# cherubicXN/neat

Measured on AMD Instinct MI355X. Metric: ray-samples/s (train step) on ABC-neat-a, higher is better.
Workload: dtype bf16; 1 GPU; C2: abc-neat-a networks, 1024 rays x 128 samples per GPU, depth samples given, train step = forward + loss + backward + Adam; rays_per_gpu=1024, samples_per_ray=128, global_rays=1024, parallelism=dp1, weights=synthetic 'rough' (seed 42), launch=hip graph replay, the whole step one launch (forward + loss + backward + Adam)

## Files before the change

neat_amd/csrc/kernels_bf16.hpp:

```cpp
#pragma once
#include "kernels.hpp"
#include "bf16_common.hpp"

namespace neat {

__device__ __forceinline__ size_t oct_index(int f, int p, int ldp) { return ((size_t)(f >> 3) * ldp + p) * 8 + (f & 7); }

struct SegH { const void* p; int rows; int bf16; };

struct LayerArgsH {
  SegH in[2];
  int Kpad;
  const uint4* Wp;
  const float* bias;
  int bias_rot, bias_n;
  int N, NT;
  int ldp;
  void* out0; void* out1;
  int out0_bf16, out1_bf16, n_split, accumulate;
  const u16* aux0; const u16* aux1;
  const u16* padfill_oct;
  const float* padfill; int padfill_rows;
};

// ... 626 lines not shown
      if (fast) {
        const int p = pb + bpg * 8;
        uint4 raw[8];
#pragma unroll
        for (int t = 0; t < 8; ++t) raw[t] = (okr && p + t < pend) ? rawl[t * 64 + lane] : make_uint4(0u, 0u, 0u, 0u);
        w2_transpose(raw, blk);
      } else {
        w2_rows_f32(pr, isA, row0, pb + bpg * 8, a.ldp, pend, blk);
      }
      unsigned char* dst = (isA ? As : Bs) + (boct * 8) * HLD + bpg * 16;
#pragma unroll
      for (int f = 0; f < 8; ++f) *reinterpret_cast<uint4*>(dst + f * HLD) = blk[f];
      if (bias_now) {
#pragma unroll
        for (int f = 0; f < 8; ++f) {
          const unsigned w4[4] = {blk[f].x, blk[f].y, blk[f].z, blk[f].w};
          float t = 0.0f;
#pragma unroll
          for (int j = 0; j < 4; ++j) t += bf_lo(w4[j]) + bf_hi(w4[j]);
          rsum[f] += t;
        }
      }
      __syncthreads();
      if (st + 1 < nsteps) W2_ISSUE(pr, pb + HBP);
      else if (q == 0 && a.npairs > 1) W2_ISSUE(a.pair[1], pbeg);
      const unsigned char* ap = As + (wr + (lane & 31)) * HLD + (lane >> 5) * 16;
      const unsigned char* bp = Bs + (wc + (lane & 31)) * HLD + (lane >> 5) * 16;
#pragma unroll
      for (int s = 0; s < HBP / 16; ++s) {
        uint4 av[2], bv[4];
#pragma unroll
        for (int i = 0; i < 2; ++i) av[i] = *reinterpret_cast<const uint4*>(ap + i * 32 * HLD + s * 32);
#pragma unroll
        for (int j = 0; j < 4; ++j) bv[j] = *reinterpret_cast<const uint4*>(bp + j * 32 * HLD + s * 32);
#pragma unroll
        for (int i = 0; i < 2; ++i) {
          if (!liveR[i]) continue;
#pragma unroll
          for (int j = 0; j < 4; ++j)
            if (liveC[j])
              acc[i][j] = NEAT_MFMA16(*reinterpret_cast<bf16x8*>(&av[i]), *reinterpret_cast<bf16x8*>(&bv[j]), acc[i][j], 0, 0, 0);
        }
      }
      __syncthreads();
    }
  }
#undef W2_ISSUE
#undef W2_SEG
#undef W2_FAST
  float* dstp = a.partial + (size_t)blockIdx.y * a.split_stride;
#pragma unroll
  for (int i = 0; i < 2; ++i) {
    if (!liveR[i]) continue;
#pragma unroll
    for (int r = 0; r < 16; ++r) {
      const int n = n0 + wr + 32 * i + (r & 3) + 8 * (r >> 2) + 4 * (lane >> 5);
      if (n >= a.N) continue;
#pragma unroll
      for (int j = 0; j < 4; ++j) {
        const int k = k0 + wc + 32 * j + (lane & 31);
        if (liveC[j] && k < a.Kt) dstp[(size_t)n * a.row_stride + k] = acc[i][j][r];
      }
    }
  }
  if (do_bias && isA) {
#pragma unroll
    for (int f = 0; f < 8; ++f) {
      float v = rsum[f];
      v += __shfl_xor(v, 1); v += __shfl_xor(v, 2); v += __shfl_xor(v, 4);
      if (bpg == 0 && row0 + f < a.N) dstp[(size_t)(row0 + f) * a.row_stride + a.bias_col] = v;
    }
  }
}

struct OctPackJob { const float* src; int rows; u16* dst; };
struct OctPackArgs { OctPackJob job[4]; int njobs, ldp; };
__global__ void oct_pack_kernel(OctPackArgs a) {
  const int p = blockIdx.x * blockDim.x + threadIdx.x;
  if (p >= a.ldp) return;
#pragma unroll
  for (int j = 0; j < 4; ++j) {
    if (j >= a.njobs) break;
    const OctPackJob jb = a.job[j];
    for (int o = 0; o * 8 < jb.rows; ++o) {
      float v[8];
#pragma unroll
      for (int e = 0; e < 8; ++e) v[e] = (o * 8 + e < jb.rows) ? jb.src[(size_t)(o * 8 + e) * a.ldp + p] : 0.0f;
      reinterpret_cast<uint4*>(jb.dst)[(size_t)o * a.ldp + p] = make_uint4(pack2(v[0], v[1]), pack2(v[2], v[3]), pack2(v[4], v[5]), pack2(v[6], v[7]));
    }
  }
}

struct BwdPrologueArgs {
  const float* sc_r; const float* sc_a; const float* extra_rm; const float* mask; const float* d_tail_rm;
  const float* cot_slot; const float* cot_slot_a;
  int P, ldp, P_main;
  const float* x_fm; const float* E;
  float* gh; float* Eh;
  u16* Ebf; u16* Ebf4; u16* Ehbf; u16* Ehbf4;
  const float* dbeta_ray; int R; const float* beta_ptr; float* dbeta;
};
__global__ __launch_bounds__(256) void bwd_prologue_kernel(BwdPrologueArgs a) {
  if (a.dbeta && blockIdx.x == gridDim.x - 1) { beta_grad_body(a.dbeta_ray, a.R, a.beta_ptr, a.dbeta); return; }
  const int p = blockIdx.x * blockDim.x + threadIdx.x;
  if (p >= a.ldp) return;
  const size_t ldp = (size_t)a.ldp;
  const float ext_scale = cot_scale_of(a.cot_slot);
  const float rho_a = a.cot_slot_a ? ext_scale / cot_scale_of(a.cot_slot_a) : 1.0f;
  const float keep = (p < a.P) ? 1.0f - (a.mask ? a.mask[p] : 0.0f) : 0.0f;
  float eh[40], ev[40];
#pragma unroll
  for (int c = 0; c < 3; ++c) {
    float v = 0.0f;
    if (p < a.P_main) {
      if (a.sc_r) v += a.sc_r[(size_t)(30 + c) * ldp + p];
      if (a.sc_a) v += a.sc_a[(size_t)(6 + c) * ldp + p] * rho_a;
      if (a.extra_rm) v += a.extra_rm[p * 3 + c] * ext_scale;
    } else if (p < a.P && a.d_tail_rm) {
      v = a.d_tail_rm[(p - a.P_main) * 3 + c] * ext_scale;
    }
    const float gc = v * keep;
    a.gh[(size_t)c * ldp + p] = gc;
    const float xc = a.x_fm[(size_t)c * ldp + p];
    eh[c] = gc;
    float f = 1.0f;
#pragma unroll
    for (int k = 0; k < 6; ++k) {
      eh[3 + 6 * k + c] = f * __cosf(xc * f) * gc;
      eh[6 + 6 * k + c] = -f * __sinf(xc * f) * gc;
      f *= 2.0f;
    }
  }
  eh[39] = 0.0f; ev[39] = 0.0f;
#pragma unroll
  for (int j = 0; j < 39; ++j) { a.Eh[(size_t)j * ldp + p] = eh[j]; ev[j] = a.E[(size_t)j * ldp + p]; }
  auto octet = [](const float (&v)[40], int r0) {
    float t[8];
#pragma unroll
    for (int e = 0; e < 8; ++e) t[e] = (r0 + e < 39) ? v[r0 + e] : 0.0f;
    return make_uint4(pack2(t[0], t[1]), pack2(t[2], t[3]), pack2(t[4], t[5]), pack2(t[6], t[7]));
  };
#pragma unroll
  for (int o = 0; o < 5; ++o) {
    reinterpret_cast<uint4*>(a.Ebf)[(size_t)o * ldp + p] = octet(ev, 8 * o);
    reinterpret_cast<uint4*>(a.Ehbf)[(size_t)o * ldp + p] = octet(eh, 8 * o);
  }
#pragma unroll
  for (int o = 0; o < 4; ++o) {
    reinterpret_cast<uint4*>(a.Ebf4)[(size_t)o * ldp + p] = octet(ev, 7 + 8 * o);
    reinterpret_cast<uint4*>(a.Ehbf4)[(size_t)o * ldp + p] = octet(eh, 7 + 8 * o);
  }
}

#ifndef NEAT_W3_ABLATE
#define NEAT_W3_ABLATE 0
#endif
constexpr int W3T = 512, W3P = 32, W3NS = 4;
template <int NCB> struct W3Cfg {
  static constexpr int QA = 8, QB = 2 * NCB;
  static constexpr int STAGE = (QA + QB) * 2048;
  static constexpr int LDS = W3NS * STAGE;
  static constexpr int QPW = NCB == 5 ? 3 : 2;
  static constexpr int G = 2 * QPW;
};
constexpr int W3_STAGE = W3Cfg<4>::STAGE;
constexpr int W3_LDS_BYTES = W3Cfg<4>::LDS;
constexpr int W3_SLOTS = 12;
struct WgradArgsH3 {
  const unsigned short* A[W3_SLOTS]; const unsigned short* B[W3_SLOTS]; int rowsA[W3_SLOTS];
  const unsigned short* B2[W3_SLOTS];
  int splitB, octsB;
  int npairs, N, K, P, ldp, chunk;
  float* partial; size_t row_stride, split_stride; int col_off, bias_col;
  int nt_loads;
  int interleave;
  int nprob; size_t prob_stride;
};
typedef short v4s16 __attribute__((ext_vector_type(4)));

template <int NCB>
__global__ __launch_bounds__(W3T, 2) void wgrad_kernel_h3(WgradArgsH3 a) {
  typedef W3Cfg<NCB> C;
  extern __shared__ __attribute__((aligned(16))) unsigned char w3lds[];
  typedef __attribute__((address_space(3))) void* lds_ptr;
  typedef __attribute__((address_space(3))) v4s16* lds_v4;
  typedef const __attribute__((address_space(1))) void* gbl_ptr;
  const int tid = threadIdx.x, lane = tid & 63, wave = tid >> 6;
  const int wr = (wave >> 1) * 64, wc = (wave & 1) * 32 * NCB;
  const int nsplit = gridDim.y;
  const int pstep = a.interleave ? nsplit * W3P : W3P;
  const int pbeg = a.interleave ? blockIdx.y * W3P : blockIdx.y * a.chunk;
  const int pend = a.interleave ? a.P : min(a.P, pbeg + a.chunk);
  const int nsteps = a.interleave ? ((a.P + W3P - 1) / W3P - (int)blockIdx.y + nsplit - 1) / nsplit : (pend - pbeg + W3P - 1) / W3P;
  const int prob = a.nprob > 1 ? (int)blockIdx.x : 0;
  const int T = nsteps * a.npairs;
  bool liveR[2], liveC[NCB];
#pragma unroll
  for (int i = 0; i < 2; ++i) liveR[i] = wr + 32 * i < a.N;
#pragma unroll
  for (int j = 0; j < NCB; ++j) liveC[j] = wc + 32 * j < a.K;
  f32x16 acc[2][NCB];
#pragma unroll
  for (int i = 0; i < 2; ++i)
#pragma unroll
    for (int j = 0; j < NCB; ++j)
#pragma unroll
      for (int r = 0; r < 16; ++r) acc[i][j][r] = 0.0f;
  float rsum[2] = {0.0f, 0.0f};

  const int dl_oct = lane & 3, dl_pt = lane >> 2;
  const unsigned lds_base = (unsigned)(size_t)(lds_ptr)w3lds;
  const unsigned short* opbase[2][C::QPW]; const unsigned short* opbase2[2]; int opmax[2][C::QPW]; int opq[C::QPW]; bool opB[C::QPW];
#pragma unroll
  for (int hq = 0; hq < C::QPW; ++hq) {
    const int g = min(C::QPW * wave + hq, C::QA + C::QB - 1);
    opB[hq] = g >= C::QA; opq[hq] = opB[hq] ? g - C::QA : g;
  }
#pragma unroll
  for (int q = 0; q < 2; ++q) {
    const int idx = prob * a.npairs + q;
    const unsigned short* pA = a.A[0]; const unsigned short* pB = a.B[0]; const unsigned short* p2 = a.B2[0];
    int rA = a.rowsA[0];
#pragma unroll
    for (int k = 1; k < W3_SLOTS; ++k)
      if (idx == k) { pA = a.A[k]; pB = a.B[k]; p2 = a.B2[k]; rA = a.rowsA[k]; }
    opbase2[q] = p2;
#pragma unroll
    for (int hq = 0; hq < C::QPW; ++hq) { opbase[q][hq] = opB[hq] ? pB : pA; opmax[q][hq] = opB[hq] ? a.octsB - 1 : (rA + 7) / 8 - 1; }
  }
  auto issue = [&](int tau) {
    const int q = tau >= nsteps ? 1 : 0;
    const int st = tau - q * nsteps;
    if (NEAT_W3_ABLATE == 4) return;
    const unsigned short* base2 = q ? opbase2[1] : opbase2[0];
    const unsigned stage = lds_base + (tau % W3NS) * C::STAGE;
#pragma unroll
    for (int hq = 0; hq < C::QPW; ++hq) {
      const unsigned short* base = q ? opbase[1][hq] : opbase[0][hq];
      const int maxoct = q ? opmax[1][hq] : opmax[0][hq];
      const int oct = min(4 * opq[hq] + dl_oct, maxoct);
      const bool second = opB[hq] && oct >= a.splitB;
      const uint4* seg = reinterpret_cast<const uint4*>(second ? base2 : base) + (size_t)(second ? oct - a.splitB : oct) * a.ldp;
      const int g = min(C::QPW * wave + hq, C::QA + C::QB - 1);
#ifndef NEAT_W3_SKIP_SURPLUS
#define NEAT_W3_SKIP_SURPLUS 1
#endif
      if constexpr (NEAT_W3_SKIP_SURPLUS && 8 * C::QPW > C::QA + C::QB) { if (C::QPW * wave + hq >= C::QA + C::QB) continue; }
#pragma unroll
      for (int i = 0; i < 2; ++i) {
        const int p = pbeg + st * pstep + 16 * i + dl_pt;
        const uint4* src = seg + p;
        const unsigned dst = __builtin_amdgcn_readfirstlane(stage + g * 2048 + i * 1024);
        unsigned keep;
        if (a.nt_loads)
          asm volatile("s_mov_b32 %0, m0\n\ts_mov_b32 m0, %2\n\ts_nop 0\n\tglobal_load_lds_dwordx4 %1, off nt\n\ts_mov_b32 m0, %0"
                       : "=&s"(keep) : "v"(src), "s"(dst) : "memory");
        else
          asm volatile("s_mov_b32 %0, m0\n\ts_mov_b32 m0, %2\n\ts_nop 0\n\tglobal_load_lds_dwordx4 %1, off\n\ts_mov_b32 m0, %0"
                       : "=&s"(keep) : "v"(src), "s"(dst) : "memory");
      }
    }
  };
#pragma unroll
  for (int t = 0; t < W3NS - 1; ++t)
    if (t < T) issue(t);

  const int G = lane >> 4, li = lane & 15;
  const int frag_off = ((8 * (G >> 1) + (li >> 2)) * 64) + (G & 1) * 32 + (li & 3) * 8;
  const bool do_bias = a.bias_col >= 0 && wc == 0;

  for (int tau = 0; tau < T; ++tau) {
    if (tau + 2 < T) { if (C::G == 4) asm volatile("s_waitcnt vmcnt(8)\n\ts_barrier" ::: "memory"); else asm volatile("s_waitcnt vmcnt(12)\n\ts_barrier" ::: "memory"); }
    else if (tau + 1 < T) { if (C::G == 4) asm volatile("s_waitcnt vmcnt(4)\n\ts_barrier" ::: "memory"); else asm volatile("s_waitcnt vmcnt(6)\n\ts_barrier" ::: "memory"); }
    else asm volatile("s_waitcnt vmcnt(0)\n\ts_barrier" ::: "memory");
    if (tau + W3NS - 1 < T) issue(tau + W3NS - 1);
    const unsigned char* slot = w3lds + (tau % W3NS) * C::STAGE;
    const int st = tau >= nsteps ? tau - nsteps : tau;
    const int pb = pbeg + st * pstep;
    const bool tail = pb + W3P > pend;
    const bool bias_now = do_bias && tau < nsteps;
#pragma unroll
    for (int s2 = 0; s2 < W3P / 16; ++s2) {
      uint4 av[2], bv[NCB];
#pragma unroll
      for (int i = 0; i < 2; ++i) {
        if (NEAT_W3_ABLATE == 2) { av[i] = make_uint4(lane, tau, i, s2); continue; }
        const unsigned char* ap = slot + ((wr >> 5) + i) * 2048 + s2 * 1024 + frag_off;
        const v4s16 lo = __builtin_amdgcn_ds_read_tr16_b64_v4i16((lds_v4)(ap));
        const v4s16 hi = __builtin_amdgcn_ds_read_tr16_b64_v4i16((lds_v4)(ap + 256));
        av[i] = make_uint4(((const unsigned*)&lo)[0], ((const unsigned*)&lo)[1], ((const unsigned*)&hi)[0], ((const unsigned*)&hi)[1]);
      }
#pragma unroll
      for (int j = 0; j < NCB; ++j) {
        if (NEAT_W3_ABLATE == 2) { bv[j] = make_uint4(lane, tau, j, s2); continue; }
        const unsigned char* bp = slot + C::QA * 2048 + ((wc >> 5) + j) * 2048 + s2 * 1024 + frag_off;
        const v4s16 lo = __builtin_amdgcn_ds_read_tr16_b64_v4i16((lds_v4)(bp));
        const v4s16 hi = __builtin_amdgcn_ds_read_tr16_b64_v4i16((lds_v4)(bp + 256));
        bv[j] = make_uint4(((const unsigned*)&lo)[0], ((const unsigned*)&lo)[1], ((const unsigned*)&hi)[0], ((const unsigned*)&hi)[1]);
      }
      if (tail) {
        const int p0 = pb + 16 * s2 + 8 * (G >> 1);
        auto mask4 = [&](uint4& v) {
          unsigned w4[4] = {v.x, v.y, v.z, v.w};
#pragma unroll
          for (int e = 0; e < 4; ++e) {
            const bool k0 = p0 + 2 * e < pend, k1 = p0 + 2 * e + 1 < pend;
            w4[e] = (k0 ? (w4[e] & 0x0000FFFFu) : 0u) | (k1 ? (w4[e] & 0xFFFF0000u) : 0u);
          }
          v = make_uint4(w4[0], w4[1], w4[2], w4[3]);
        };
#pragma unroll
        for (int i = 0; i < 2; ++i) mask4(av[i]);
#pragma unroll
        for (int j = 0; j < NCB; ++j) mask4(bv[j]);
      }
      if (bias_now) {
#pragma unroll
        for (int i = 0; i < 2; ++i) {
          const unsigned w4[4] = {av[i].x, av[i].y, av[i].z, av[i].w};
          float t = rsum[i];
#pragma unroll
          for (int e = 0; e < 4; ++e) { t += bf_lo(w4[e]); t += bf_hi(w4[e]); }
          asm volatile("" : "+v"(t));
          rsum[i] = t;
        }
      }
#pragma unroll
      for (int i = 0; i < 2; ++i) {
        if (!liveR[i]) continue;
#pragma unroll
        for (int j = 0; j < NCB; ++j)
          if (liveC[j]) {
            if (NEAT_W3_ABLATE == 1) { asm volatile("" :: "v"(av[i].x), "v"(av[i].w), "v"(bv[j].x), "v"(bv[j].w)); continue; }
            acc[i][j] = NEAT_MFMA16(*reinterpret_cast<bf16x8*>(&av[i]), *reinterpret_cast<bf16x8*>(&bv[j]), acc[i][j], 0, 0, 0);
          }
      }
    }
  }
  float* dstp = a.partial + (size_t)prob * a.prob_stride + (size_t)blockIdx.y * a.split_stride;
  auto put = [&](float* q, float v) {
    if (NEAT_W3_ABLATE == 3 && v != 123.0f) return;
    *q = v;
  };
#pragma unroll
  for (int i = 0; i < 2; ++i) {
    if (!liveR[i]) continue;
#pragma unroll
    for (int r = 0; r < 16; ++r) {
      const int n = wr + 32 * i + (r & 3) + 8 * (r >> 2) + 4 * (lane >> 5);
      if (n >= a.N) continue;
#pragma unroll
      for (int j = 0; j < NCB; ++j) {
        const int k = wc + 32 * j + (lane & 31);
        if (liveC[j] && k < a.K) put(dstp + (size_t)n * a.row_stride + a.col_off + k, acc[i][j][r]);
      }
    }
  }
  if (do_bias) {
#pragma unroll
    for (int i = 0; i < 2; ++i) {
      float v = rsum[i];
      v += __shfl_xor(v, 32);
      const int n = wr + 32 * i + (lane & 31);
      if (lane < 32 && n < a.N) put(dstp + (size_t)n * a.row_stride + a.bias_col, v);
    }
  }
}

struct PackDesc2 {
  int layer, transpose, N, K, Kpad, NT;
  int s0, s0p, off0, off1;
  int rot;
  float scale; int offset; int blk0; int bf16;
  int lo;
};
constexpr int MAXPACKS2 = 48;
struct PackArgs2 { NetPtrs net; const float* rowscale; int row_off[NLAYERS + 1]; PackDesc2 d[MAXPACKS2]; int npacks; float* out; };

__device__ __forceinline__ float packed_weight(const PackDesc2& d, const float* v, const float* rs, int O, int I, int n, int k) {
  if (!v || n >= d.N || k >= d.K) return 0.0f;
  const int po = d.transpose ? k : n;
  const int pj = d.transpose ? n : k;
  if (po >= O) return 0.0f;
  const int o = (po + d.rot) % O;
  int i;
  if (pj < d.s0p) { if (pj >= d.s0) return 0.0f; i = d.off0 + pj; }
  else { i = d.off1 + (pj - d.s0p); if (pj - d.s0p >= I - d.s0) return 0.0f; }
  if (i >= I) return 0.0f;
  return v[(size_t)o * I + i] * rs[o] * d.scale;
}

__global__ __launch_bounds__(WG) void pack_kernel2(PackArgs2 a) {
  int pk = 0;
  while (pk + 1 < a.npacks && (int)blockIdx.x >= a.d[pk + 1].blk0) ++pk;
  const PackDesc2 d = a.d[pk];
  const int nt = blockIdx.x - d.blk0;
  const int O = a.net.O[d.layer], I = a.net.I[d.layer];
  const float* v = a.net.v[d.layer];
  const float* rs = a.rowscale + a.row_off[d.layer];
  if (d.bf16) {
    const int KS = d.Kpad >> 4;
    uint4* out = reinterpret_cast<uint4*>(a.out + d.offset) + (size_t)nt * KS * 64;
    for (int e = blockIdx.y * WG + threadIdx.x; e < KS * 64; e += WG * gridDim.y) {
      const int s = e >> 6, ln = e & 63;
      const int n = nt * 32 + (ln & 31), kb = 16 * s + 8 * (ln >> 5);
      float w[8];
#pragma unroll
      for (int t = 0; t < 8; ++t) w[t] = packed_weight(d, v, rs, O, I, n, kb + t);
      if (d.lo) {
#pragma unroll
        for (int t = 0; t < 8; ++t) w[t] -= bf2f(f2bf(w[t]));
      }
      out[e] = make_uint4(pack2(w[0], w[1]), pack2(w[2], w[3]), pack2(w[4], w[5]), pack2(w[6], w[7]));
    }
  } else {
    const int KS = d.Kpad >> 1;
    float* out = a.out + d.offset + (size_t)nt * KS * 64;
    for (int e = blockIdx.y * WG + threadIdx.x; e < KS * 64; e += WG * gridDim.y) {
      const int s = e >> 6, ln = e & 63;
      out[e] = packed_weight(d, v, rs, O, I, nt * 32 + (ln & 31), 2 * s + (ln >> 5));
    }
  }
}

__global__ void adjoint_seed_kernel_h(const float* __restrict__ v8, const float* __restrict__ rs8, const u16* __restrict__ h8,
                                      int ldp, u16* __restrict__ u7) {
  const int p = blockIdx.x * blockDim.x + threadIdx.x;
  const int oct = blockIdx.y;
  if (p >= ldp) return;
  const size_t idx = ((size_t)oct * ldp + p) * 8;
  const uint4 hv = *reinterpret_cast<const uint4*>(h8 + idx);
  const unsigned hw[4] = {hv.x, hv.y, hv.z, hv.w};
  unsigned o[4];
#pragma unroll
  for (int j = 0; j < 4; ++j) {
    const float w0 = v8[oct * 8 + 2 * j] * rs8[0], w1 = v8[oct * 8 + 2 * j + 1] * rs8[0];
    o[j] = pack2(w0 * dphi_fast(bf_lo(hw[j])), w1 * dphi_fast(bf_hi(hw[j])));
  }
  *reinterpret_cast<uint4*>(u7 + idx) = make_uint4(o[0], o[1], o[2], o[3]);
}

__global__ void oct_to_rm_kernel(const u16* __restrict__ src, int P, int C, int ldp, float* __restrict__ dst, int ldc, int col0,
                                 const u16* __restrict__ srclo = nullptr) {
  const int p = blockIdx.x * blockDim.x + threadIdx.x, o = blockIdx.y;
  if (p >= P) return;
  const uint4 v = reinterpret_cast<const uint4*>(src)[(size_t)o * ldp + p];
  uint4 vl = make_uint4(0u, 0u, 0u, 0u);
  if (srclo) vl = reinterpret_cast<const uint4*>(srclo)[(size_t)o * ldp + p];
  const unsigned w4[4] = {v.x, v.y, v.z, v.w}, l4[4] = {vl.x, vl.y, vl.z, vl.w};
  float* d = dst + (size_t)p * ldc + col0 + o * 8;
#pragma unroll
  for (int j = 0; j < 4; ++j) {
    if (o * 8 + 2 * j < C) d[2 * j] = bf_lo(w4[j]) + bf_lo(l4[j]);
    if (o * 8 + 2 * j + 1 < C) d[2 * j + 1] = bf_hi(w4[j]) + bf_hi(l4[j]);
  }
}
__global__ void export_out8_kernel(const float* __restrict__ sdfraw, const u16* __restrict__ src, const u16* __restrict__ srclo, int P, int ldp,
                                   float* __restrict__ out257, float* __restrict__ feat) {
  const int p = blockIdx.x * blockDim.x + threadIdx.x, o = blockIdx.y;
  if (p >= P) return;
  const uint4 v = reinterpret_cast<const uint4*>(src)[(size_t)o * ldp + p];
  uint4 vl = make_uint4(0u, 0u, 0u, 0u);
  if (srclo) vl = reinterpret_cast<const uint4*>(srclo)[(size_t)o * ldp + p];
  const unsigned w4[4] = {v.x, v.y, v.z, v.w}, l4[4] = {vl.x, vl.y, vl.z, vl.w};
  float f[8];
#pragma unroll
  for (int j = 0; j < 4; ++j) { f[2 * j] = bf_lo(w4[j]) + bf_lo(l4[j]); f[2 * j + 1] = bf_hi(w4[j]) + bf_hi(l4[j]); }
  if (out257) {
    float* d = out257 + (size_t)p * 257 + 1 + o * 8;
#pragma unroll
    for (int j = 0; j < 8; ++j) d[j] = f[j];
    if (o == 0) out257[(size_t)p * 257] = sdfraw[p];
  }
  if (feat) {
    float* d = feat + (size_t)p * 256 + o * 8;
#pragma unroll
    for (int j = 0; j < 8; ++j) d[j] = f[j];
  }
}
__global__ void rm_to_oct_kernel(const float* __restrict__ src, int P, int C, int ldp, u16* __restrict__ dst, u16* __restrict__ dstlo = nullptr) {
  const int p = blockIdx.x * blockDim.x + threadIdx.x;
  if (p >= ldp) return;
  const int Cp = (C + 7) & ~7;
  for (int c = 0; c < Cp; ++c) {
    const float v = (p < P && c < C) ? src[(size_t)p * C + c] : 0.0f;
    const u16 h = f2bf(v);
    dst[oct_index(c, p, ldp)] = h;
    if (dstlo) dstlo[oct_index(c, p, ldp)] = f2bf(v - bf2f(h));
  }
}
__global__ void fm_col_to_rm_kernel(const float* __restrict__ src, int P, float* __restrict__ dst, int ldc, int col) {
  const int p = blockIdx.x * blockDim.x + threadIdx.x;
  if (p < P) dst[(size_t)p * ldc + col] = src[p];
}
// ... 3 lines not shown
```

neat_amd/csrc/kernels_dw.hpp:

```cpp
#pragma once
#include "kernels_bf16.hpp"

namespace neat {

struct LayerArgsDW {
  LayerArgsWS w;
  const u16* auxA2; int auxA_split;
  int rowsA;
  int P;
  uint4* partial;
  float* pscale;
  float* pbias;
  int ablate;
};

constexpr int DW_MAXSEG = 4;
struct LayerArgsDWSeg { LayerArgsDW l[DW_MAXSEG]; int n; };

constexpr int DW_XLDS = 1024;
constexpr int DW_WG_UINT4 = 8 * 8 * 2 * 64;
#ifndef DW_VALU_PER_MFMA
#define DW_VALU_PER_MFMA 14
#endif

// ... 149 lines not shown
          dacc[i * 4 + j] = NEAT_MFMA16(*reinterpret_cast<const bf16x8*>(&av[i]), *reinterpret_cast<const bf16x8*>(&bv[j]), dacc[i * 4 + j], 0, 0, 0);
    };
    f32x16 acc;
    auto chain = [&]() {
#pragma unroll
      for (int r = 0; r < 16; ++r) acc[r] = 0.0f;
      const unsigned bfrag_e = (hi5 * WSP + (l31 ^ (hi5 << 2))) * 16;
      const unsigned bfrag_o = (hi5 * WSP + (l31 ^ ((2 + hi5) << 2))) * 16;
#pragma unroll
      for (int ks = 0; ks < 16; ++ks) {
        const uint4 bv = *reinterpret_cast<const uint4*>(slot + ((ks & 1) ? bfrag_o : bfrag_e) + ks * (2 * WSP * 16));
        acc = NEAT_MFMA16(*reinterpret_cast<const bf16x8*>(&wreg[ks]), *reinterpret_cast<const bf16x8*>(&bv), acc, 0, 0, 0);
      }
    };
    const int p = tile * WSP + (int)l31;
    auto epi_half = [&](int j, bool fullrows, const uint4* fa = nullptr, const uint4* fb = nullptr) {
      float sp = 0.0f;
      if (C::HAS_S) sp = *reinterpret_cast<const float*>(slot + EXTRA + wave * 256 + l31 * 4);
      uint2 pk0[2], pk1[2];
#pragma unroll
      for (int qq = 0; qq < 2; ++qq) {
        const int q = 2 * j + qq;
        pk0[qq] = make_uint2(0u, 0u); pk1[qq] = make_uint2(0u, 0u);
        const int n0 = wave * 32 + 8 * q + 4 * (int)hi5;
        if (!fullrows && fa) {
#pragma unroll
          for (int e = 0; e < 4; ++e) {
            const int t = qq * 4 + e;
            dacc[t] = NEAT_MFMA16(*reinterpret_cast<const bf16x8*>(&fa[t >> 2]), *reinterpret_cast<const bf16x8*>(&fb[t & 3]), dacc[t], 0, 0, 0);
          }
        }
        if (!fullrows && wave * 32 + 8 * q >= Npad) continue;
        const unsigned eoff = dma_off + q * (WSP * 16) + ((l31 ^ ((unsigned)q << 2)) * 16) + hi5 * 8;
        const uint2 r0v = *reinterpret_cast<const uint2*>(slot + AUX0 + eoff);
        const uint2 r1v = *reinterpret_cast<const uint2*>(slot + AUX1 + eoff);
        const float x0[4] = {bf_lo(r0v.x), bf_hi(r0v.x), bf_lo(r0v.y), bf_hi(r0v.y)};
        const float x1[4] = {bf_lo(r1v.x), bf_hi(r1v.x), bf_lo(r1v.y), bf_hi(r1v.y)};
        float o0[4], o1[4];
        float4 b8 = make_float4(0.f, 0.f, 0.f, 0.f);
        if (EPI == EPI_BWD8) b8 = *reinterpret_cast<const float4*>(w8 + n0);
        const float bias8q[4] = {b8.x, b8.y, b8.z, b8.w};
#pragma unroll
        for (int e = 0; e < 4; ++e) {
          const float v = acc[4 * q + e];
          if (fa && fullrows) {
            const int t = qq * 4 + e;
            dacc[t] = NEAT_MFMA16(*reinterpret_cast<const bf16x8*>(&fa[t >> 2]), *reinterpret_cast<const bf16x8*>(&fb[t & 3]), dacc[t], 0, 0, 0);
          }
          float r0 = 0.0f, r1 = 0.0f;
          if (TANK) { const float sg = dphi_fast(x0[e]); r0 = v * sg; r1 = v * x1[e] * (100.0f * (1.0f - sg)); }
          else if (EPI == EPI_BWD) r0 = v * dphi_fast(x0[e]) + x1[e];
          else if (EPI == EPI_BWD8) r0 = (v + bias8q[e] * sp) * dphi_fast(x0[e]) + x1[e];
          if (!fullrows && n0 + e >= a.N) {
            r0 = 0.0f; r1 = 0.0f;
            if (C::HAS_PF && n0 + e < a.N + 7)
              r0 = bf2f(*reinterpret_cast<const u16*>(slot + EXTRA + l31 * 16 + (n0 + e - a.N) * 2));
          }
          o0[e] = r0; o1[e] = r1;
        }
        pk0[qq] = make_uint2(pack2(o0[0], o0[1]), pack2(o0[2], o0[3]));
        if (TANK) pk1[qq] = make_uint2(pack2(o1[0], o1[1]), pack2(o1[2], o1[3]));
      }
      const int ob = wave * 32 + 16 * j;
      if (!fullrows && ob >= Npad) return;
      const int oct = (ob >> 3) + (int)hi5;
      const unsigned oidx = ((unsigned)oct * (unsigned)a.ldp + (unsigned)p) * 8u;
      const bool in_range = fullrows || oct * 8 < Npad;
      typedef unsigned v2u_t __attribute__((ext_vector_type(2)));
      typedef unsigned v4u_t __attribute__((ext_vector_type(4)));
      {
        const v2u_t s0 = __builtin_amdgcn_permlane32_swap(pk0[0].x, pk0[1].x, false, false);
        const v2u_t s1 = __builtin_amdgcn_permlane32_swap(pk0[0].y, pk0[1].y, false, false);
        if (in_range) {
          const v4u_t v = {s0.x, s1.x, s0.y, s1.y};
          *reinterpret_cast<v4u_t*>(a.out0 + oidx) = v;
        }
      }
      if (TANK) {
        const v2u_t s0 = __builtin_amdgcn_permlane32_swap(pk1[0].x, pk1[1].x, false, false);
        const v2u_t s1 = __builtin_amdgcn_permlane32_swap(pk1[0].y, pk1[1].y, false, false);
        if (in_range) *reinterpret_cast<uint4*>(a.out1 + oidx) = make_uint4(s0.x, s1.x, s0.y, s1.y);
      }
    };
    uint4 av[2], bv[4];
    load_frags(0, av, bv);
    if (!FULL || tail) mask_frags(0, av, bv, tail);
    if (live) chain();
    __builtin_amdgcn_sched_barrier(0);
    dw_mma(av, bv, false);
    epi_half(0, FULL, av, bv);
    __builtin_amdgcn_sched_barrier(0);
    load_frags(1, av, bv);
    if (!FULL || tail) mask_frags(1, av, bv, tail);
    dw_mma(av, bv, false);
    epi_half(1, FULL, av, bv);
    __builtin_amdgcn_sched_barrier(0);
  }

  const int lane = lane0;
  float amax = 0.0f;
#pragma unroll
  for (int j = 0; j < 8; ++j)
#pragma unroll
    for (int r = 0; r < 16; ++r) amax = fmaxf(amax, fabsf(dacc[j][r]));
#pragma unroll
  for (int off = 32; off > 0; off >>= 1) amax = fmaxf(amax, __shfl_xor(amax, off));
  unsigned ex = (__float_as_uint(amax) >> 23) & 255u;
  ex = ex < 15u ? 15u : (ex > 253u ? 253u : ex);
  const float sc = __uint_as_float((268u - ex) << 23);
  uint4* dst = d.partial + (size_t)blockIdx.x * DW_WG_UINT4 + (size_t)wave * (8 * 2 * 64) + lane;
  typedef _Float16 h2_t __attribute__((ext_vector_type(2)));
#pragma unroll
  for (int j = 0; j < 8; ++j)
#pragma unroll
    for (int hf = 0; hf < 2; ++hf) {
      if (d.ablate & 4) continue;
      unsigned w4[4];
#pragma unroll
      for (int e = 0; e < 4; ++e) {
        const f32x2_t v = {dacc[j][8 * hf + 2 * e] * sc, dacc[j][8 * hf + 2 * e + 1] * sc};
        w4[e] = __builtin_bit_cast(unsigned, __builtin_convertvector(v, h2_t));
      }
#ifndef NEAT_DW_NT_PART
#define NEAT_DW_NT_PART 0
#endif
      if (NEAT_DW_NT_PART) {
        typedef unsigned v4u_t __attribute__((ext_vector_type(4)));
        const v4u_t wv = {w4[0], w4[1], w4[2], w4[3]};
        __builtin_nontemporal_store(wv, reinterpret_cast<v4u_t*>(dst + (j * 2 + hf) * 64));
      } else dst[(j * 2 + hf) * 64] = make_uint4(w4[0], w4[1], w4[2], w4[3]);
    }
  if (lane == 0) d.pscale[blockIdx.x * 8 + wave] = __uint_as_float((ex - 14u) << 23);
  if (!TANK && BIAS) {
#pragma unroll
    for (int i = 0; i < 2; ++i) {
      const float t = bsum[i] + __shfl_xor(bsum[i], 32);
      if (lane < 32) d.pbias[blockIdx.x * 256 + wr + 32 * i + lane] = t;
    }
  }
  }
}

struct DwGatherJob {
  const uint4* partial; const float* pscale; const float* pbias;
  const uint4* partial2; const float* pscale2;
  int nwg, transposed;
  float* out; size_t row_stride, split_stride; int split0;
  int bias_col;
  int rows, cols;
  const float* xrow; int xrow_n; size_t xrow_stride;
};
constexpr int DW_MAXJOBS = 16;
struct DwGatherArgs { DwGatherJob job[DW_MAXJOBS]; };

__global__ __launch_bounds__(256) void dw_gather_kernel(DwGatherArgs) {
  const DwGatherJob* tab = (const DwGatherJob*)__builtin_amdgcn_kernarg_segment_ptr();
  const DwGatherJob jb = tab[blockIdx.z];
  const int nsub = gridDim.y, sub = blockIdx.y;
  const int per = (jb.nwg + nsub - 1) / nsub;
  const int g0 = sub * per, g1 = min(jb.nwg, g0 + per);
  const int pos = blockIdx.x * 256 + threadIdx.x;
  const int lane = pos & 63, hf = (pos >> 6) & 1, j = (pos >> 7) & 7, wave = pos >> 10;
  float acc[8] = {0.f, 0.f, 0.f, 0.f, 0.f, 0.f, 0.f, 0.f};
  typedef _Float16 h2_t __attribute__((ext_vector_type(2)));
#pragma unroll
  for (int set = 0; set < 2; ++set) {
    const uint4* part = set ? jb.partial2 : jb.partial;
    const float* psc = set ? jb.pscale2 : jb.pscale;
    if (!part) break;
#pragma unroll 8
    for (int g = g0; g < g1; ++g) {
      typedef unsigned v4u_t __attribute__((ext_vector_type(4)));
      const v4u_t v = __builtin_nontemporal_load(reinterpret_cast<const v4u_t*>(part + (size_t)g * DW_WG_UINT4 + pos));
      const float s = psc[g * 8 + wave];
      const unsigned w4[4] = {v.x, v.y, v.z, v.w};
#pragma unroll
      for (int e = 0; e < 4; ++e) {
        const h2_t h = __builtin_bit_cast(h2_t, w4[e]);
        acc[2 * e] += (float)h.x * s;
        acc[2 * e + 1] += (float)h.y * s;
      }
    }
  }
  float* out = jb.out + (size_t)(jb.split0 + sub) * jb.split_stride;
  const int col = 128 * (wave & 1) + 32 * (j & 3) + (lane & 31);
#pragma unroll
  for (int e = 0; e < 8; ++e) {
    const int r = 8 * hf + e;
    const int row = 64 * (wave >> 1) + 32 * (j >> 2) + (r & 3) + 8 * (r >> 2) + 4 * (lane >> 5);
    const int n = jb.transposed ? col : row, k = jb.transposed ? row : col;
    if (n < jb.rows && k < jb.cols) out[(size_t)n * jb.row_stride + k] = acc[e];
  }
  if (jb.bias_col >= 0 && blockIdx.x == 0) {
    const int n = threadIdx.x;
    float t = 0.0f;
    if (jb.pbias)
      for (int g = g0; g < g1; ++g) t += jb.pbias[g * 256 + n];
    if (n < jb.rows) out[(size_t)n * jb.row_stride + jb.bias_col] = t;
  }
  if (jb.xrow && blockIdx.x == 1) {
    const int perx = (jb.xrow_n + nsub - 1) / nsub;
    const int b0 = sub * perx, b1 = min(jb.xrow_n, b0 + perx);
    for (int k = threadIdx.x; k <= jb.cols; k += 256) {
      float t = 0.0f;
#pragma unroll 8
      for (int b = b0; b < b1; ++b) t += jb.xrow[(size_t)b * jb.xrow_stride + k];
      out[(size_t)jb.rows * jb.row_stride + k] = t;
    }
  }
}

}
```

Baseline: 50.29 million ray-samples/s.

## Rebalance wgrad LDS staging loads across waves and batch dw_gather loads

The wgrad kernel's global-to-LDS staging is redistributed. Each wave now issues one row-half per quad across NK k-slices, replacing the old per-wave quad groups with surplus-skip logic, and the counted vmcnt waits are rewritten to match per-wave issue counts. The dw_gather kernel now issues eight nontemporal loads and scale loads ahead of a sched_barrier before accumulating, to raise memory-level parallelism, and it derives the wave index from blockIdx. Ablation and timestamp probe hooks are moved into an optional header; this adds risk of wrong vmcnt counts if the per-wave issue counts are miscounted.

```diff
diff --git a/neat_amd/csrc/kernels_bf16.hpp b/neat_amd/csrc/kernels_bf16.hpp
--- a/neat_amd/csrc/kernels_bf16.hpp
+++ b/neat_amd/csrc/kernels_bf16.hpp
@@ -802,16 +802,25 @@
   }
 }
 
-#ifndef NEAT_W3_ABLATE
-#define NEAT_W3_ABLATE 0
+#ifdef NEAT_W3_PROBE
+#include "w3_probe.hpp"
+#else
+#define W3_ABL_NO_DMA
+#define W3_ABL_FRAG(v, i)
+#define W3_ABL_MFMA(x, y)
+#define W3_ABL_PUT(v)
+#define W3_STAMP_DECL
+#define W3_STAMP(i)
+#define W3_STAMP_REPORT
 #endif
 constexpr int W3T = 512, W3P = 32, W3NS = 4;
 template <int NCB> struct W3Cfg {
   static constexpr int QA = 8, QB = 2 * NCB;
   static constexpr int STAGE = (QA + QB) * 2048;
   static constexpr int LDS = W3NS * STAGE;
-  static constexpr int QPW = NCB == 5 ? 3 : 2;
-  static constexpr int G = 2 * QPW;
+  static constexpr int NH = 2 * (QA + QB);
+  static constexpr int NK = (NH + 7) / 8;
+  static constexpr int XW = NH - 8 * (NK - 1);
 };
 constexpr int W3_STAGE = W3Cfg<4>::STAGE;
 constexpr int W3_LDS_BYTES = W3Cfg<4>::LDS;
@@ -860,12 +869,7 @@
 
   const int dl_oct = lane & 3, dl_pt = lane >> 2;
   const unsigned lds_base = (unsigned)(size_t)(lds_ptr)w3lds;
-  const unsigned short* opbase[2][C::QPW]; const unsigned short* opbase2[2]; int opmax[2][C::QPW]; int opq[C::QPW]; bool opB[C::QPW];
-#pragma unroll
-  for (int hq = 0; hq < C::QPW; ++hq) {
-    const int g = min(C::QPW * wave + hq, C::QA + C::QB - 1);
-    opB[hq] = g >= C::QA; opq[hq] = opB[hq] ? g - C::QA : g;
-  }
+  const unsigned short* opA[2]; const unsigned short* opB[2]; const unsigned short* opbase2[2]; int maxA[2];
 #pragma unroll
   for (int q = 0; q < 2; ++q) {
     const int idx = prob * a.npairs + q;
@@ -874,43 +878,37 @@
 #pragma unroll
     for (int k = 1; k < W3_SLOTS; ++k)
       if (idx == k) { pA = a.A[k]; pB = a.B[k]; p2 = a.B2[k]; rA = a.rowsA[k]; }
-    opbase2[q] = p2;
-#pragma unroll
-    for (int hq = 0; hq < C::QPW; ++hq) { opbase[q][hq] = opB[hq] ? pB : pA; opmax[q][hq] = opB[hq] ? a.octsB - 1 : (rA + 7) / 8 - 1; }
-  }
+    opA[q] = pA; opB[q] = pB; opbase2[q] = p2; maxA[q] = (rA + 7) / 8 - 1;
+  }
+  const int wave_u = __builtin_amdgcn_readfirstlane(wave);
+  const bool more = C::XW == 8 || wave_u < C::XW;
   auto issue = [&](int tau) {
     const int q = tau >= nsteps ? 1 : 0;
     const int st = tau - q * nsteps;
-    if (NEAT_W3_ABLATE == 4) return;
-    const unsigned short* base2 = q ? opbase2[1] : opbase2[0];
+    W3_ABL_NO_DMA
     const unsigned stage = lds_base + (tau % W3NS) * C::STAGE;
-#pragma unroll
-    for (int hq = 0; hq < C::QPW; ++hq) {
-      const unsigned short* base = q ? opbase[1][hq] : opbase[0][hq];
-      const int maxoct = q ? opmax[1][hq] : opmax[0][hq];
-      const int oct = min(4 * opq[hq] + dl_oct, maxoct);
-      const bool second = opB[hq] && oct >= a.splitB;
-      const uint4* seg = reinterpret_cast<const uint4*>(second ? base2 : base) + (size_t)(second ? oct - a.splitB : oct) * a.ldp;
-      const int g = min(C::QPW * wave + hq, C::QA + C::QB - 1);
-#ifndef NEAT_W3_SKIP_SURPLUS
-#define NEAT_W3_SKIP_SURPLUS 1
-#endif
-      if constexpr (NEAT_W3_SKIP_SURPLUS && 8 * C::QPW > C::QA + C::QB) { if (C::QPW * wave + hq >= C::QA + C::QB) continue; }
-#pragma unroll
-      for (int i = 0; i < 2; ++i) {
-        const int p = pbeg + st * pstep + 16 * i + dl_pt;
-        const uint4* src = seg + p;
-        const unsigned dst = __builtin_amdgcn_readfirstlane(stage + g * 2048 + i * 1024);
-        unsigned keep;
-        if (a.nt_loads)
-          asm volatile("s_mov_b32 %0, m0\n\ts_mov_b32 m0, %2\n\ts_nop 0\n\tglobal_load_lds_dwordx4 %1, off nt\n\ts_mov_b32 m0, %0"
-                       : "=&s"(keep) : "v"(src), "s"(dst) : "memory");
-        else
-          asm volatile("s_mov_b32 %0, m0\n\ts_mov_b32 m0, %2\n\ts_nop 0\n\tglobal_load_lds_dwordx4 %1, off\n\ts_mov_b32 m0, %0"
-                       : "=&s"(keep) : "v"(src), "s"(dst) : "memory");
-      }
+    const int p = pbeg + st * pstep + 16 * (wave & 1) + dl_pt;
+#pragma unroll
+    for (int k = 0; k < C::NK; ++k) {
+      if (k == C::NK - 1 && !more) continue;
+      const bool isB = k >= 2;
+      const int quad = (wave >> 1) + 4 * (isB ? k - 2 : k);
+      const unsigned short* base = isB ? (q ? opB[1] : opB[0]) : (q ? opA[1] : opA[0]);
+      const int maxoct = isB ? a.octsB - 1 : (q ? maxA[1] : maxA[0]);
+      const int oct = min(4 * quad + dl_oct, maxoct);
+      const bool second = isB && oct >= a.splitB;
+      const uint4* src = reinterpret_cast<const uint4*>(second ? (q ? opbase2[1] : opbase2[0]) : base) + (size_t)(second ? oct - a.splitB : oct) * a.ldp + p;
+      const unsigned dst = __builtin_amdgcn_readfirstlane(stage + ((wave >> 1) + 4 * k) * 2048 + (wave & 1) * 1024);
+      unsigned keep;
+      if (a.nt_loads)
+        asm volatile("s_mov_b32 %0, m0\n\ts_mov_b32 m0, %2\n\ts_nop 0\n\tglobal_load_lds_dwordx4 %1, off nt\n\ts_mov_b32 m0, %0"
+                     : "=&s"(keep) : "v"(src), "s"(dst) : "memory");
+      else
+        asm volatile("s_mov_b32 %0, m0\n\ts_mov_b32 m0, %2\n\ts_nop 0\n\tglobal_load_lds_dwordx4 %1, off\n\ts_mov_b32 m0, %0"
+                     : "=&s"(keep) : "v"(src), "s"(dst) : "memory");
     }
   };
+  static_assert(C::NK == 4 || C::NK == 5 || C::NK == 3, "counted waits are written out for these stage shapes");
 #pragma unroll
   for (int t = 0; t < W3NS - 1; ++t)
     if (t < T) issue(t);
@@ -919,10 +917,23 @@
   const int frag_off = ((8 * (G >> 1) + (li >> 2)) * 64) + (G & 1) * 32 + (li & 3) * 8;
   const bool do_bias = a.bias_col >= 0 && wc == 0;
 
+  W3_STAMP_DECL
   for (int tau = 0; tau < T; ++tau) {
-    if (tau + 2 < T) { if (C::G == 4) asm volatile("s_waitcnt vmcnt(8)\n\ts_barrier" ::: "memory"); else asm volatile("s_waitcnt vmcnt(12)\n\ts_barrier" ::: "memory"); }
-    else if (tau + 1 < T) { if (C::G == 4) asm volatile("s_waitcnt vmcnt(4)\n\ts_barrier" ::: "memory"); else asm volatile("s_waitcnt vmcnt(6)\n\ts_barrier" ::: "memory"); }
-    else asm volatile("s_waitcnt vmcnt(0)\n\ts_barrier" ::: "memory");
+    W3_STAMP(0);
+    {
+      const int newer = tau + 2 < T ? 2 : tau + 1 < T ? 1 : 0;
+#ifdef W3_WAIT_STAMPED
+#define W3_WAIT(n) W3_WAIT_STAMPED(n)
+#else
+#define W3_WAIT(n) asm volatile("s_waitcnt vmcnt(" #n ")\n\ts_barrier" ::: "memory")
+#endif
+      if (newer == 0) W3_WAIT(0);
+      else if (C::NK == 4) { if (newer == 2) W3_WAIT(8); else W3_WAIT(4); }
+      else if (C::NK == 5) { if (more) { if (newer == 2) W3_WAIT(10); else W3_WAIT(5); } else { if (newer == 2) W3_WAIT(8); else W3_WAIT(4); } }
+      else { if (more) { if (newer == 2) W3_WAIT(6); else W3_WAIT(3); } else { if (newer == 2) W3_WAIT(4); else W3_WAIT(2); } }
+#undef W3_WAIT
+    }
+    W3_STAMP(2);
     if (tau + W3NS - 1 < T) issue(tau + W3NS - 1);
     const unsigned char* slot = w3lds + (tau % W3NS) * C::STAGE;
     const int st = tau >= nsteps ? tau - nsteps : tau;
@@ -934,7 +945,7 @@
       uint4 av[2], bv[NCB];
 #pragma unroll
       for (int i = 0; i < 2; ++i) {
-        if (NEAT_W3_ABLATE == 2) { av[i] = make_uint4(lane, tau, i, s2); continue; }
+        W3_ABL_FRAG(av[i], i)
         const unsigned char* ap = slot + ((wr >> 5) + i) * 2048 + s2 * 1024 + frag_off;
         const v4s16 lo = __builtin_amdgcn_ds_read_tr16_b64_v4i16((lds_v4)(ap));
         const v4s16 hi = __builtin_amdgcn_ds_read_tr16_b64_v4i16((lds_v4)(ap + 256));
@@ -942,7 +953,7 @@
       }
 #pragma unroll
       for (int j = 0; j < NCB; ++j) {
-        if (NEAT_W3_ABLATE == 2) { bv[j] = make_uint4(lane, tau, j, s2); continue; }
+        W3_ABL_FRAG(bv[j], j)
         const unsigned char* bp = slot + C::QA * 2048 + ((wc >> 5) + j) * 2048 + s2 * 1024 + frag_off;
         const v4s16 lo = __builtin_amdgcn_ds_read_tr16_b64_v4i16((lds_v4)(bp));
         const v4s16 hi = __builtin_amdgcn_ds_read_tr16_b64_v4i16((lds_v4)(bp + 256));
@@ -981,15 +992,17 @@
 #pragma unroll
         for (int j = 0; j < NCB; ++j)
           if (liveC[j]) {
-            if (NEAT_W3_ABLATE == 1) { asm volatile("" :: "v"(av[i].x), "v"(av[i].w), "v"(bv[j].x), "v"(bv[j].w)); continue; }
+            W3_ABL_MFMA(av[i], bv[j])
             acc[i][j] = NEAT_MFMA16(*reinterpret_cast<bf16x8*>(&av[i]), *reinterpret_cast<bf16x8*>(&bv[j]), acc[i][j], 0, 0, 0);
           }
       }
     }
-  }
+    W3_STAMP(3);
+  }
+  W3_STAMP_REPORT
   float* dstp = a.partial + (size_t)prob * a.prob_stride + (size_t)blockIdx.y * a.split_stride;
   auto put = [&](float* q, float v) {
-    if (NEAT_W3_ABLATE == 3 && v != 123.0f) return;
+    W3_ABL_PUT(v)
     *q = v;
   };
 #pragma unroll
diff --git a/neat_amd/csrc/kernels_dw.hpp b/neat_amd/csrc/kernels_dw.hpp
--- a/neat_amd/csrc/kernels_dw.hpp
+++ b/neat_amd/csrc/kernels_dw.hpp
@@ -325,6 +325,19 @@
 };
 constexpr int DW_MAXJOBS = 16;
 struct DwGatherArgs { DwGatherJob job[DW_MAXJOBS]; };
+constexpr int DWG_UN = 8;
+#ifndef NEAT_DWG_STAMPS
+#define NEAT_DWG_STAMPS 0
+#endif
+#if NEAT_DWG_STAMPS
+#define DWG_STAMP_BEGIN const unsigned long long dwg_t0 = __builtin_amdgcn_s_memtime();
+#define DWG_STAMP_END if (blockIdx.x == 0 && blockIdx.y == 0 && blockIdx.z == 0 && threadIdx.x == 0) { float keep_ = 0.f; \
+    for (int e = 0; e < 8; ++e) keep_ += acc[e]; \
+    printf("dwg stamp: %llu cycles for %d partials x %d sets (%g)\n", __builtin_amdgcn_s_memtime() - dwg_t0, g1 - g0, jb.partial2 ? 2 : 1, keep_); }
+#else
+#define DWG_STAMP_BEGIN
+#define DWG_STAMP_END
+#endif
 
 __global__ __launch_bounds__(256) void dw_gather_kernel(DwGatherArgs) {
   const DwGatherJob* tab = (const DwGatherJob*)__builtin_amdgcn_kernarg_segment_ptr();
@@ -333,19 +346,18 @@
   const int per = (jb.nwg + nsub - 1) / nsub;
   const int g0 = sub * per, g1 = min(jb.nwg, g0 + per);
   const int pos = blockIdx.x * 256 + threadIdx.x;
-  const int lane = pos & 63, hf = (pos >> 6) & 1, j = (pos >> 7) & 7, wave = pos >> 10;
+  const int lane = pos & 63, hf = (pos >> 6) & 1, j = (pos >> 7) & 7;
+  const int wave = blockIdx.x >> 2;
   float acc[8] = {0.f, 0.f, 0.f, 0.f, 0.f, 0.f, 0.f, 0.f};
   typedef _Float16 h2_t __attribute__((ext_vector_type(2)));
+  typedef unsigned v4u_t __attribute__((ext_vector_type(4)));
+  DWG_STAMP_BEGIN
 #pragma unroll
   for (int set = 0; set < 2; ++set) {
     const uint4* part = set ? jb.partial2 : jb.partial;
     const float* psc = set ? jb.pscale2 : jb.pscale;
     if (!part) break;
-#pragma unroll 8
-    for (int g = g0; g < g1; ++g) {
-      typedef unsigned v4u_t __attribute__((ext_vector_type(4)));
-      const v4u_t v = __builtin_nontemporal_load(reinterpret_cast<const v4u_t*>(part + (size_t)g * DW_WG_UINT4 + pos));
-      const float s = psc[g * 8 + wave];
+    auto add = [&](const v4u_t& v, const float s) {
       const unsigned w4[4] = {v.x, v.y, v.z, v.w};
 #pragma unroll
       for (int e = 0; e < 4; ++e) {
@@ -353,8 +365,23 @@
         acc[2 * e] += (float)h.x * s;
         acc[2 * e + 1] += (float)h.y * s;
       }
+    };
+    int g = g0;
+    for (; g + DWG_UN <= g1; g += DWG_UN) {
+      v4u_t v[DWG_UN]; float sc[DWG_UN];
+#pragma unroll
+      for (int u = 0; u < DWG_UN; ++u) {
+        v[u] = __builtin_nontemporal_load(reinterpret_cast<const v4u_t*>(part + (size_t)(g + u) * DW_WG_UINT4 + pos));
+        sc[u] = psc[(g + u) * 8 + wave];
+      }
+      __builtin_amdgcn_sched_barrier(0);
+#pragma unroll
+      for (int u = 0; u < DWG_UN; ++u) add(v[u], sc[u]);
     }
-  }
+    for (; g < g1; ++g)
+      add(__builtin_nontemporal_load(reinterpret_cast<const v4u_t*>(part + (size_t)g * DW_WG_UINT4 + pos)), psc[g * 8 + wave]);
+  }
+  DWG_STAMP_END
   float* out = jb.out + (size_t)(jb.split0 + sub) * jb.split_stride;
   const int col = 128 * (wave & 1) + 32 * (j & 3) + (lane & 31);
 #pragma unroll
diff --git a/neat_amd/csrc/w3_probe.hpp b/neat_amd/csrc/w3_probe.hpp
--- /dev/null
+++ b/neat_amd/csrc/w3_probe.hpp
@@ -0,0 +1,27 @@
+#pragma once
+#ifndef NEAT_W3_ABLATE
+#define NEAT_W3_ABLATE 0
+#endif
+#ifndef NEAT_W3_STAMPS
+#define NEAT_W3_STAMPS 0
+#endif
+#define W3_ABL_NO_DMA if (NEAT_W3_ABLATE == 4) return;
+#define W3_ABL_FRAG(v, i) if (NEAT_W3_ABLATE == 2) { v = make_uint4(lane, tau, i, s2); continue; }
+#define W3_ABL_MFMA(fa_, fb_) if (NEAT_W3_ABLATE == 1) { asm volatile("" :: "v"(fa_.x), "v"(fa_.w), "v"(fb_.x), "v"(fb_.w)); continue; }
+#define W3_ABL_PUT(v) if (NEAT_W3_ABLATE == 3 && v != 123.0f) return;
+#if NEAT_W3_STAMPS
+#ifndef W3_STAMP_T0
+#define W3_STAMP_T0 6
+#endif
+constexpr int W3_STAMP_N = 4;
+#define W3_STAMP_DECL unsigned long long w3st[W3_STAMP_N][4] = {};
+#define W3_STAMP(i) do { if (blockIdx.x == 0 && blockIdx.y == 0) { const unsigned long long t_ = __builtin_amdgcn_s_memtime(); \
+    _Pragma("unroll") for (int k_ = 0; k_ < W3_STAMP_N; ++k_) if (tau == W3_STAMP_T0 + k_) w3st[k_][i] = t_; } } while (0)
+#define W3_WAIT_STAMPED(n) do { asm volatile("s_waitcnt vmcnt(" #n ")" ::: "memory"); W3_STAMP(1); asm volatile("s_barrier" ::: "memory"); } while (0)
+#define W3_STAMP_REPORT if (blockIdx.x == 0 && blockIdx.y == 0 && lane == 0) { _Pragma("unroll") for (int k_ = 0; k_ < W3_STAMP_N; ++k_) \
+    printf("w3stamp ncb %d T %d wave %d tau %d : %llu %llu %llu %llu\n", NCB, T, wave, W3_STAMP_T0 + k_, w3st[k_][0], w3st[k_][1], w3st[k_][2], w3st[k_][3]); }
+#else
+#define W3_STAMP_DECL
+#define W3_STAMP(i)
+#define W3_STAMP_REPORT
+#endif
```

New measurement: 50.49 million ray-samples/s (median of 6 runs). Within noise of the previous version (+0.4%).
